# lucastrefezza/quadruplet-sentence-transformer

Measured on AMD Instinct MI355X. Metric: quadruplets/sec (seq_len=128, all-MiniLM-L6-v2) training step, higher is better.
Workload: dtype bf16; 1 GPU; all-MiniLM-L6-v2 dims (random-init), 64 quadruplets/GPU x 1 GPU, seq_len=128, fwd + gamma-quadruplet loss + bwd + clip + AdamW, dropout 0.1 on hidden states and attention probabilities as the reference's train() mode (BASELINE.json configs[1]); global_batch=64, seq_len=128, parallelism=dp1, precision=bf16 MFMA operands, fp32 accumulate/residual/LN/softmax/loss/optimizer, launch=eager

## Files before the change

include/qst_kernels.h:

```cpp
#pragma once
#include <stddef.h>
#include <stdint.h>

#ifdef __cplusplus
extern "C" {
#endif

enum {
    QST_EPI_BF16 = 0,
    QST_EPI_F32_RESID = 1,
    QST_EPI_GELU = 2,
    QST_EPI_GELU_BWD = 3,
    QST_EPI_F32_RESID_BF16 = 4,
    QST_EPI_GELU_MX = 5,
    QST_EPI_GELU_MX_TRAIN = 6
};

typedef struct {
    const uint32_t* state;
    uint32_t site;
    uint32_t thr16;
} QstDrop;
#define QST_DROP_SITE_EMBED 0xE0u
#define QST_DROP_SITE_ATTN_OUT(layer) (4u * (uint32_t)(layer) + 0u)
// ... 73 lines not shown
    int32_t order;
} QstTnGroup;
int qst_gemm_tn_group(const QstTnGroup* grp, void* stream);
int qst_tn_group_ranges(const QstTnGroup* grp, int32_t* row_begin);

int qst_gemm8_stagger(int cycles);
int qst_gemm8_ln_store(int mode);
int qst_gemm_nt8_supported(const QstGemmArgs* a, int epi);
int qst_gemm_nt8(const QstGemmArgs* a, int epi, int tile, void* stream);
int qst_gemm_tn8_group(const QstTnGroup* grp, void* stream);
int qst_gemm_nt8_f8(const QstGemmArgs* a, int epi, int tile, void* stream);
int qst_gemm8_mode(int mode);

int qst_embed_ln_fwd(const int64_t* ids, const int64_t* type_ids, const int32_t* pos_ids,
                     const float* word_emb, const float* pos_emb, const float* type_emb,
                     const float* gamma, const float* beta, float eps, int M, int H,
                     float* y, void* y_bf16, void* xhat_bf16, float* rstd, void* stream);
int qst_embed_ln_fwd_drop(const int64_t* ids, const int64_t* type_ids, const int32_t* pos_ids,
                          const float* word_emb, const float* pos_emb, const float* type_emb,
                          const float* gamma, const float* beta, float eps, int M, int H,
                          float* y, void* y_bf16, void* xhat_bf16, float* rstd, const QstDrop* drop, void* stream);
int qst_ln_fwd(const float* s, const float* gamma, const float* beta, float eps, int M, int H,
               float* y, void* y_bf16, void* xhat_bf16, float* rstd, void* stream);
int qst_ln_fwd_mx(const float* s, const float* gamma, const float* beta, float eps, int M, int H,
                  float* y, void* y_bf16, void* yq, void* ys, void* stream);
int qst_embed_ln_fwd_mx(const int64_t* ids, const int64_t* type_ids, const int32_t* pos_ids,
                        const float* word_emb, const float* pos_emb, const float* type_emb,
                        const float* gamma, const float* beta, float eps, int M, int H,
                        float* y, void* y_bf16, void* yq, void* ys, void* stream);
int qst_ln_fwd_mx_train(const float* s, const float* gamma, const float* beta, float eps, int M, int H, float* y,
                        void* y_bf16, void* xhat_bf16, float* rstd, void* yq, void* ys, void* stream);
int qst_embed_ln_fwd_mx_train(const int64_t* ids, const int64_t* type_ids, const int32_t* pos_ids,
                              const float* word_emb, const float* pos_emb, const float* type_emb,
                              const float* gamma, const float* beta, float eps, int M, int H, float* y,
                              void* y_bf16, void* xhat_bf16, float* rstd, void* yq, void* ys,
                              const QstDrop* drop , void* stream);
size_t qst_ln_bwd_scratch_bytes(int M, int H);
int qst_ln_bwd(const float* dy, const void* xhat_bf16, const float* rstd, const float* gamma, int M, int H,
               float* ds, void* ds_bf16, float* dgamma, float* dbeta, float* scratch, void* stream);
int qst_ln_bwd_drop(const float* dy, const void* xhat_bf16, const float* rstd, const float* gamma, int M, int H,
                    float* ds, void* ds_bf16, float* dgamma, float* dbeta, float* scratch,
                    const QstDrop* drop_in, const QstDrop* drop_out, void* stream);
#define QST_LN_BATCH_MAX 32
typedef struct {
    int32_t count, H, nblocks;
    const float* partials[QST_LN_BATCH_MAX];
    float* dgamma[QST_LN_BATCH_MAX];
    float* dbeta[QST_LN_BATCH_MAX];
    int32_t nblocks_each[QST_LN_BATCH_MAX];
} QstLnReduceBatch;
int qst_ln_bwd_reduce_batch(const QstLnReduceBatch* b, void* stream);
int qst_embed_bwd(const float* ds, const int64_t* ids, const int64_t* type_ids, const int32_t* pos_ids,
                  int nseq, int L, int H, int num_types, float* dword, float* dpos, float* dtype_, void* stream);
int qst_position_ids(const int64_t* ids, int nseq, int L, int arch, int pad_id, int32_t* pos_ids, void* stream);
int qst_forward_prologue(const int64_t* ids, int nseq, int L, int arch, int pad_id, int32_t* pos_ids,
                         uint32_t* drop_state, uint32_t* drop_snapshot, void* stream);

#define QST_POOL_CLS 1
#define QST_POOL_MAX 2
#define QST_POOL_MEAN 4
#define QST_POOL_MEAN_SQRT 8
#define QST_POOL_WMEAN 16
#define QST_POOL_ALL 31
int qst_pool_fwd(const float* tok, const int64_t* mask, int nseq, int L, int H, int mode, int normalize,
                 float* emb, float* pooled, int32_t* argmax, void* stream);
int qst_pool_bwd(const float* demb, const float* pooled, const int32_t* argmax, const int64_t* mask, int nseq, int L, int H,
                 int mode, int normalize, float* dtok, void* stream);

int qst_attention_fwd(const void* qkv, const int64_t* mask, const float* rel_pos, int nseq, int L, int A, int d,
                      void* ctx, float* lse, void* stream);
int qst_attention_bwd(const void* qkv, const void* ctx, const void* dctx, const float* lse, const int64_t* mask,
                      const float* rel_bias, int nseq, int L, int A, int d, void* dqkv, float* drel,
                      float* delta_scratch, void* stream);
typedef struct {
    const void* qkv; const int64_t* mask; const float* rel_pos;
    int32_t nseq, L, A, d;
    void* ctx; float* lse;
    const void* dctx; void* dqkv; float* drel; float* delta_scratch;
    int32_t force_split;
    QstDrop drop;
} QstAttnDesc;
int qst_attention_fwd_ex(const QstAttnDesc* a, void* stream);
int qst_attention_bwd_ex(const QstAttnDesc* a, void* stream);

int qst_rel_bucket_host(int rel, int num_buckets, int max_distance);
int qst_rel_bias_fwd(const float* table, const int32_t* lut, int A, int L, float* rel_bias, void* stream);
int qst_rel_bias_bwd(const float* drel, const int32_t* lut, int buckets, int A, int L, float* dtable, void* stream);
int qst_rel_pos_fwd(const float* table, const int32_t* lut, int A, int L, float* rel_pos, void* stream);
int qst_rel_pos_bwd(const float* drel_pos, const int32_t* lut, int buckets, int A, int L, float* dtable, void* stream);

int qst_gemm_nt_x3(const QstGemmArgs* a, int epi, void* stream);
int qst_gemm_tn_x3(const QstGemmArgs* a, void* stream);
int qst_attention_fwd_x3(const float* qkv, const int64_t* mask, const float* rel_bias, int nseq, int L, int A, int d,
                         float* ctx, void* stream);
int qst_attention_fwd_x3_drop(const float* qkv, const int64_t* mask, const float* rel_bias, int nseq, int L, int A, int d,
                              float* ctx, const QstDrop* drop, void* stream);
int qst_transpose_f32(const float* src, int R, int C, int ld_src, float* dst, int ld_dst, void* stream);
int qst_gelu_f32(const float* u, int64_t n, float* h, void* stream);
int qst_gelu_bwd_f32(const float* dh, const float* u, int64_t n, float* du, void* stream);
int qst_colsum_f32(const float* x, int M, int N, int ld, float* out, void* stream);
int qst_embed_sum_f32(const int64_t* ids, const int64_t* type_ids, const int32_t* pos_ids, const float* word_emb,
                      const float* pos_emb, const float* type_emb, int M, int H, float* s, void* stream);
int qst_ln_bwd_f32(const float* dy, const float* prenorm, const float* gamma, float eps, int M, int H, float* ds,
                   float* dgamma, float* dbeta, void* stream);
int qst_attention_bwd_f32(const float* qkv, const float* ctx, const float* dctx, const int64_t* mask, const float* rel_bias,
                          int nseq, int L, int A, int d, float* dqkv, float* drel_bias, void* stream);
int qst_attention_bwd_f32_drop(const float* qkv, const float* ctx, const float* dctx, const int64_t* mask, const float* rel_bias,
                               int nseq, int L, int A, int d, float* dqkv, float* drel_bias, const QstDrop* drop, void* stream);
size_t qst_attention_bwd_x3_scratch_bytes(int nseq, int L, int A);
int qst_attention_bwd_x3(const float* qkv, const float* ctx, const float* dctx, const int64_t* mask, const float* rel_bias,
                         int nseq, int L, int A, int d, float* dqkv, float* drel_bias, void* scratch, const QstDrop* drop,
                         void* stream);
int qst_dropout_apply_f32(const QstDrop* d, const float* in, const float* resid, int64_t n, float* out, void* stream);

int qst_topk_rows(const float* scores, int64_t ld, const int64_t* index_map, int nrows, int n, int k,
                  float* out_scores, int64_t* out_index, void* stream);

int qst_topk_merge_rows(const float* scores, int64_t ld, int nrows, int n, int64_t col_base, int64_t row_base,
                        int exclude_self, float max_score, int k, float* run_scores, int64_t* run_index, void* stream);

size_t qst_topk_stream_workspace_bytes(int nq, int chunk, int dim);
int qst_topk_stream(const float* queries, const float* corpus, int nq, int nc, int dim, int k, int mode, int chunk,
                    int64_t query_base, int64_t corpus_base, int exclude_self, float max_score,
                    float* run_scores, int64_t* run_index, void* workspace, size_t workspace_bytes, void* stream);

size_t qst_community_workspace_bytes(int n, int chunk, int dim);
int qst_community_count(const float* emb, int n, int dim, float threshold, int chunk, int32_t* counts,
                        uint8_t* self_member, void* workspace, size_t workspace_bytes, void* stream);
int qst_community_members(const float* emb, int n, int dim, float threshold, int chunk, int row0, const int64_t* begin,
                          const int32_t* capacity, int32_t* out_index, float* out_score, int32_t* written,
                          void* workspace, size_t workspace_bytes, void* stream);
int qst_community_claim(const int64_t* begin, const int32_t* len, int ncand, const int32_t* members, int n,
                        uint8_t* taken, uint8_t* accepted, void* stream);
int qst_community_rescore(const float* emb, int n, int dim, const int32_t* rows_a, const int32_t* rows_b, int64_t count,
                          double* out, void* stream);

int qst_shadow_all(const float* params, void* shadow, const int64_t* table_dev, int nseg, int nblocks, void* stream);
int qst_shadow_matrix(const float* src, int rows, int cols, void* dst_bf16, void* dstT_bf16, void* stream);

int qst_gemm_nt_f16(const QstGemmArgs* a, int epi, void* stream);
int qst_gemm_nt_ln_f16(const QstGemmArgs* a, const QstLnEpi* ln, int mode, void* stream);
int qst_gemm_nt8_ln_supported_f16(int N);
int qst_gemm_nt8_ln_block_rows_f16(int M, int N);
int qst_gemm_nt8_ln_f16(const QstGemmArgs* a, const QstLnEpi* ln, int mode, void* stream);
int qst_gemm_nt8_ln_timeouts_f16(void);
int qst_ffn_chain_f16(const QstFfnArgs* a, const QstLnEpi* ln, int mode, void* stream);
int qst_gemm_tn_f16(const QstGemmArgs* a, void* stream);
int qst_gemm_tn_group_f16(const QstTnGroup* grp, void* stream);
int qst_gemm_nt8_supported_f16(const QstGemmArgs* a, int epi);
int qst_gemm_nt8_f16(const QstGemmArgs* a, int epi, int tile, void* stream);
int qst_gemm_tn8_group_f16(const QstTnGroup* grp, void* stream);
int qst_embed_ln_fwd_f16(const int64_t* ids, const int64_t* type_ids, const int32_t* pos_ids,
                         const float* word_emb, const float* pos_emb, const float* type_emb,
                         const float* gamma, const float* beta, float eps, int M, int H,
                         float* y, void* y_f16, void* xhat_f16, float* rstd, void* stream);
int qst_embed_ln_fwd_drop_f16(const int64_t* ids, const int64_t* type_ids, const int32_t* pos_ids,
                              const float* word_emb, const float* pos_emb, const float* type_emb,
                              const float* gamma, const float* beta, float eps, int M, int H,
                              float* y, void* y_f16, void* xhat_f16, float* rstd, const QstDrop* drop, void* stream);
int qst_ln_fwd_f16(const float* s, const float* gamma, const float* beta, float eps, int M, int H,
                   float* y, void* y_f16, void* xhat_f16, float* rstd, void* stream);
int qst_ln_bwd_f16(const float* dy, const void* xhat_f16, const float* rstd, const float* gamma, int M, int H,
                   float* ds, void* ds_f16, float* dgamma, float* dbeta, float* scratch, void* stream);
int qst_ln_bwd_drop_f16(const float* dy, const void* xhat_f16, const float* rstd, const float* gamma, int M, int H,
                        float* ds, void* ds_f16, float* dgamma, float* dbeta, float* scratch,
                        const QstDrop* drop_in, const QstDrop* drop_out, void* stream);
// ... 18 lines not shown
```

quadruplet-sentence-transformer_amd/_lib.py:

```python
from __future__ import annotations

import ctypes as C
import os
from typing import Optional

_HERE = os.path.dirname(os.path.abspath(__file__))
LIB_PATH = os.path.join(_HERE, "libqst.so")

c_i64p = C.POINTER(C.c_int64)
c_i32p = C.POINTER(C.c_int32)
c_f32p = C.POINTER(C.c_float)
vp = C.c_void_p


class QstError(RuntimeError):
    pass


class QstConfig(C.Structure):
    _fields_ = [("arch", C.c_int32), ("vocab_size", C.c_int32), ("hidden_size", C.c_int32),
                ("num_layers", C.c_int32), ("num_heads", C.c_int32), ("intermediate_size", C.c_int32),
                ("max_position", C.c_int32), ("type_vocab_size", C.c_int32), ("layer_norm_eps", C.c_float),
                ("normalize", C.c_int32), ("rel_buckets", C.c_int32), ("rel_max_distance", C.c_int32),
                ("pad_token_id", C.c_int32), ("precision", C.c_int32)]
# ... 69 lines not shown
                                vp]),
    "qst_mnrl_nested_workspace_bytes": (C.c_size_t, [C.c_int, C.c_int, C.c_int, C.c_int]),
    "qst_mnrl_nested_loss": (C.c_int, [vp, vp, C.c_int, C.c_int, C.c_int, c_i32p, c_f32p, C.c_int, C.c_float, C.c_int, vp, vp,
                                       vp, vp, vp, vp, C.c_size_t, vp]),
    "qst_batch_triplet_workspace_bytes": (C.c_size_t, [C.c_int, C.c_int]),
    "qst_batch_triplet_loss": (C.c_int, [vp, vp, C.c_int, C.c_int, C.c_int, C.c_int, C.c_float, vp, vp, vp, vp, vp, C.c_size_t,
                                         vp]),
    "qst_cosent_workspace_bytes": (C.c_size_t, [C.c_int, C.c_int]),
    "qst_cosent_loss": (C.c_int, [vp, vp, vp, C.c_int, C.c_int, C.c_int, C.c_float, vp, vp, vp, vp, vp, vp, C.c_size_t, vp]),
    "qst_embed_mse": (C.c_int, [vp, vp, C.c_int, C.c_int, vp, vp, vp, vp, vp]),
    "qst_margin_mse_loss": (C.c_int, [vp, vp, vp, vp, C.c_int, C.c_int, C.c_int, C.c_int, vp, vp, vp, vp, vp, vp, vp, vp]),
    "qst_clip_adamw_step": (C.c_int, [vp, vp, vp, vp, vp, C.c_float, C.c_float, C.c_float, C.c_float, C.c_float,
                                      C.c_float, C.c_float, C.c_int64, vp, vp, vp]),
    "qst_clip_adamw_step_joint": (C.c_int, [vp, vp, vp, vp, vp, vp, vp, vp, vp, vp, C.c_int64, C.c_float, C.c_float, C.c_float,
                                            C.c_float, C.c_float, C.c_float, C.c_float, C.c_int64, vp, vp, vp]),
    "qst_softmax_head_fwd": (C.c_int, [vp, vp, vp, vp, C.c_int, C.c_int, C.c_int, C.c_int, vp, vp]),
    "qst_softmax_head_bwd_workspace_bytes": (C.c_size_t, [C.c_int, C.c_int, C.c_int, C.c_int]),
    "qst_softmax_head_bwd": (C.c_int, [vp, vp, vp, vp, C.c_int, C.c_int, C.c_int, C.c_int, vp, vp, vp, vp, vp, C.c_size_t, vp]),
    "qst_dense_head_fwd": (C.c_int, [vp, C.c_int, vp, vp, C.c_int, C.c_int, C.c_int, C.c_int, C.c_int, vp, vp, vp]),
    "qst_dense_head_bwd_workspace_bytes": (C.c_size_t, [C.c_int, C.c_int, C.c_int]),
    "qst_dense_head_bwd": (C.c_int, [vp, C.c_int, vp, vp, vp, vp, C.c_int, C.c_int, C.c_int, C.c_int, C.c_int, vp, vp, vp, vp,
                                     C.c_size_t, vp]),
    "qst_softmax_ce": (C.c_int, [vp, vp, C.c_int, C.c_int, C.c_int64, C.c_int, vp, vp, vp, vp, vp, vp]),
    "qst_binary_eval_workspace_bytes": (C.c_size_t, [C.c_int64, C.c_int]),
    "qst_binary_eval": (C.c_int, [vp, vp, C.c_int64, C.c_int, c_i32p, vp, vp, C.c_size_t, vp]),
    "qst_rerank_scores": (C.c_int, [vp, vp, vp, C.c_int64, C.c_int64, C.c_int, C.c_int, vp, vp]),
    "qst_rerank_workspace_bytes": (C.c_size_t, [C.c_int64, C.c_int64]),
    "qst_rerank_metrics": (C.c_int, [vp, vp, vp, C.c_int64, C.c_int64, C.c_int, vp, vp, vp, C.c_size_t, vp]),
    "qst_shadow8_bytes": (C.c_int64, [C.POINTER(QstConfig)]),
    "qst_clip_adamw_step_sched": (C.c_int, [vp, vp, vp, vp, vp, C.c_float, C.c_float, C.c_float, C.c_float, C.c_float,
                                            C.c_float, C.c_float, C.c_int64, C.c_int64, vp, vp, vp, vp]),
    "qst_topk_workspace_bytes": (C.c_size_t, [C.c_int, C.c_int, C.c_int]),
    "qst_topk_scores": (C.c_int, [vp, vp, C.c_int, C.c_int, C.c_int, C.c_int, C.c_int, vp, vp, vp, C.c_size_t, vp]),
    "qst_topk_scores_capped": (C.c_int, [vp, vp, C.c_int, C.c_int, C.c_int, C.c_int, C.c_int, C.c_float, vp, vp, vp,
                                         C.c_size_t, vp]),
    "qst_score_workspace_bytes": (C.c_size_t, [C.c_int, C.c_int, C.c_int]),
    "qst_score_matrix": (C.c_int, [vp, vp, C.c_int, C.c_int, C.c_int, C.c_int, vp, C.c_int64, vp, C.c_size_t, vp]),
    "qst_gemm_nt": (C.c_int, [C.POINTER(QstGemmArgs), C.c_int, vp]),
    "qst_gemm_nt_f8": (C.c_int, [C.POINTER(QstGemmArgs), C.c_int, vp]),
    "qst_quant_mx": (C.c_int, [vp, C.c_int, C.c_int64, C.c_int, vp, vp, vp]),
    "qst_gemm_nt_ln_supported": (C.c_int, [C.c_int]),
    "qst_gemm_nt_ln": (C.c_int, [C.POINTER(QstGemmArgs), C.POINTER(QstLnEpi), C.c_int, vp]),
    "qst_gemm_nt_ln_block_rows": (C.c_int, [C.c_int]),
    "qst_gemm_nt_ln_block_rows_m": (C.c_int, [C.c_int, C.c_int]),
    "qst_gemm_nt8_ln_block_rows": (C.c_int, [C.c_int, C.c_int]),
    "qst_gemm8_stagger": (C.c_int, [C.c_int]),
    "qst_gemm8_ln_store": (C.c_int, [C.c_int]),
    "qst_gemm_nt8_ln_supported": (C.c_int, [C.c_int]),
    "qst_gemm_nt8_ln": (C.c_int, [C.POINTER(QstGemmArgs), C.POINTER(QstLnEpi), C.c_int, vp]),
    "qst_gemm_nt8_ln_timeouts": (C.c_int, []),
    "qst_gemm_nt8_f8_ln": (C.c_int, [C.POINTER(QstGemmArgs), C.POINTER(QstLnEpi), vp]),
    "qst_ffn_chain_supported": (C.c_int, [C.c_int, C.c_int]),
    "qst_ffn_chain": (C.c_int, [C.POINTER(QstFfnArgs), C.POINTER(QstLnEpi), C.c_int, vp]),
    "qst_gemm_tn": (C.c_int, [C.POINTER(QstGemmArgs), vp]),
    "qst_gemm_tn_group": (C.c_int, [C.POINTER(QstTnGroup), vp]),
    "qst_tn_group_ranges": (C.c_int, [C.POINTER(QstTnGroup), c_i32p]),
    "qst_gemm_nt8_supported": (C.c_int, [C.POINTER(QstGemmArgs), C.c_int]),
    "qst_gemm_nt8": (C.c_int, [C.POINTER(QstGemmArgs), C.c_int, C.c_int, vp]),
    "qst_gemm_tn8_group": (C.c_int, [C.POINTER(QstTnGroup), vp]),
    "qst_gemm_nt8_f8": (C.c_int, [C.POINTER(QstGemmArgs), C.c_int, C.c_int, vp]),
    "qst_gemm8_mode": (C.c_int, [C.c_int]),
    "qst_embed_ln_fwd": (C.c_int, [vp, vp, vp, vp, vp, vp, vp, vp, C.c_float, C.c_int, C.c_int, vp, vp, vp, vp, vp]),
    "qst_embed_ln_fwd_drop": (C.c_int, [vp, vp, vp, vp, vp, vp, vp, vp, C.c_float, C.c_int, C.c_int, vp, vp, vp, vp,
                                        C.POINTER(QstDrop), vp]),
    "qst_ln_fwd_mx": (C.c_int, [vp, vp, vp, C.c_float, C.c_int, C.c_int, vp, vp, vp, vp, vp]),
    "qst_embed_ln_fwd_mx": (C.c_int, [vp, vp, vp, vp, vp, vp, vp, vp, C.c_float, C.c_int, C.c_int, vp, vp, vp, vp, vp]),
    "qst_ln_fwd_mx_train": (C.c_int, [vp, vp, vp, C.c_float, C.c_int, C.c_int, vp, vp, vp, vp, vp, vp, vp]),
    "qst_embed_ln_fwd_mx_train": (C.c_int, [vp, vp, vp, vp, vp, vp, vp, vp, C.c_float, C.c_int, C.c_int, vp, vp, vp, vp, vp, vp,
                                            vp, vp]),
    "qst_ln_fwd": (C.c_int, [vp, vp, vp, C.c_float, C.c_int, C.c_int, vp, vp, vp, vp, vp]),
    "qst_ln_bwd_scratch_bytes": (C.c_size_t, [C.c_int, C.c_int]),
    "qst_ln_bwd_reduce_batch": (C.c_int, [vp, vp]),
    "qst_ln_bwd": (C.c_int, [vp, vp, vp, vp, C.c_int, C.c_int, vp, vp, vp, vp, vp, vp]),
    "qst_ln_bwd_drop": (C.c_int, [vp, vp, vp, vp, C.c_int, C.c_int, vp, vp, vp, vp, vp, C.POINTER(QstDrop), C.POINTER(QstDrop), vp]),
    "qst_embed_bwd": (C.c_int, [vp, vp, vp, vp, C.c_int, C.c_int, C.c_int, C.c_int, vp, vp, vp, vp]),
    "qst_position_ids": (C.c_int, [vp, C.c_int, C.c_int, C.c_int, C.c_int, vp, vp]),
    "qst_forward_prologue": (C.c_int, [vp, C.c_int, C.c_int, C.c_int, C.c_int, vp, vp, vp, vp]),
    "qst_pool_fwd": (C.c_int, [vp, vp, C.c_int, C.c_int, C.c_int, C.c_int, C.c_int, vp, vp, vp, vp]),
    "qst_pool_bwd": (C.c_int, [vp, vp, vp, vp, C.c_int, C.c_int, C.c_int, C.c_int, C.c_int, vp, vp]),
    "qst_attention_fwd": (C.c_int, [vp, vp, vp, C.c_int, C.c_int, C.c_int, C.c_int, vp, vp, vp]),
    "qst_attention_bwd": (C.c_int, [vp, vp, vp, vp, vp, vp, C.c_int, C.c_int, C.c_int, C.c_int, vp, vp, vp, vp]),
    "qst_attention_fwd_ex": (C.c_int, [C.POINTER(QstAttnDesc), vp]),
    "qst_attention_bwd_ex": (C.c_int, [C.POINTER(QstAttnDesc), vp]),
    "qst_dropout_multipliers": (C.c_int, [C.POINTER(QstDrop), C.c_int, C.c_int64, vp, vp]),
    "qst_abi_sizeof": (C.c_int64, [C.c_int]),
    "qst_normalize_rows": (C.c_int, [vp, C.c_int, C.c_int, vp, vp]),
    "qst_cls_head_fwd": (C.c_int, [vp, C.c_int64, C.c_int, C.c_int, vp, vp, vp, vp, C.c_int, C.c_int, C.c_int, vp, vp]),
    "qst_dropout_init": (C.c_int, [vp, C.c_uint64, vp]),
    "qst_dropout_advance": (C.c_int, [vp, vp]),
    "qst_encoder_set_dropout": (C.c_int, [vp, C.c_float, C.c_float, vp]),
    "qst_encoder_set_ffn_chain": (C.c_int, [vp, C.c_int]),
    "qst_encoder_set_ln_fusion": (C.c_int, [vp, C.c_int]),
    "qst_encoder_set_wgrad_pairs": (C.c_int, [vp, C.c_int]),
    "qst_wgrad_pairs_rule": (C.c_int, [C.POINTER(QstConfig), C.c_int]),
    "qst_wgrad_tiles": (C.c_int, [C.POINTER(QstConfig), C.c_int, C.c_int]),
    "qst_encoder_set_pooling": (C.c_int, [vp, C.c_int]),
    "qst_encoder_embedding_dim": (C.c_int, [vp]),
    "qst_transpose_f32": (C.c_int, [vp, C.c_int, C.c_int, C.c_int, vp, C.c_int, vp]),
    "qst_gelu_f32": (C.c_int, [vp, C.c_int64, vp, vp]),
    "qst_gelu_bwd_f32": (C.c_int, [vp, vp, C.c_int64, vp, vp]),
    "qst_colsum_f32": (C.c_int, [vp, C.c_int, C.c_int, C.c_int, vp, vp]),
    "qst_embed_sum_f32": (C.c_int, [vp, vp, vp, vp, vp, vp, C.c_int, C.c_int, vp, vp]),
    "qst_ln_bwd_f32": (C.c_int, [vp, vp, vp, C.c_float, C.c_int, C.c_int, vp, vp, vp, vp]),
    "qst_attention_bwd_f32": (C.c_int, [vp, vp, vp, vp, vp, C.c_int, C.c_int, C.c_int, C.c_int, vp, vp, vp]),
    "qst_attention_bwd_f32_drop": (C.c_int, [vp, vp, vp, vp, vp, C.c_int, C.c_int, C.c_int, C.c_int, vp, vp, vp, vp]),
    "qst_attention_bwd_x3_scratch_bytes": (C.c_size_t, [C.c_int, C.c_int, C.c_int]),
    "qst_attention_bwd_x3": (C.c_int, [vp, vp, vp, vp, vp, C.c_int, C.c_int, C.c_int, C.c_int, vp, vp, vp, vp, vp]),
    "qst_dropout_apply_f32": (C.c_int, [vp, vp, vp, C.c_int64, vp, vp]),
    "qst_comm_unique_id": (C.c_int, [vp]),
    "qst_comm_init": (C.c_int, [C.c_int, C.c_int, vp, C.POINTER(vp)]),
    "qst_allreduce_bucket": (C.c_int, [vp, vp, C.c_int64, C.c_int, vp]),
    "qst_comm_rank": (C.c_int, [vp]),
    "qst_comm_world": (C.c_int, [vp]),
    "qst_comm_destroy": (None, [vp]),
    "qst_comm_last_error": (C.c_char_p, []),
    "qst_rel_bucket_host": (C.c_int, [C.c_int, C.c_int, C.c_int]),
    "qst_rel_bias_fwd": (C.c_int, [vp, vp, C.c_int, C.c_int, vp, vp]),
    "qst_rel_bias_bwd": (C.c_int, [vp, vp, C.c_int, C.c_int, C.c_int, vp, vp]),
    "qst_rel_pos_fwd": (C.c_int, [vp, vp, C.c_int, C.c_int, vp, vp]),
    "qst_rel_pos_bwd": (C.c_int, [vp, vp, C.c_int, C.c_int, C.c_int, vp, vp]),
    "qst_topk_rows": (C.c_int, [vp, C.c_int64, vp, C.c_int, C.c_int, C.c_int, vp, vp, vp]),
    "qst_topk_merge_rows": (C.c_int, [vp, C.c_int64, C.c_int, C.c_int, C.c_int64, C.c_int64, C.c_int, C.c_float, C.c_int,
                                      vp, vp, vp]),
    "qst_topk_stream_workspace_bytes": (C.c_size_t, [C.c_int, C.c_int, C.c_int]),
    "qst_topk_stream": (C.c_int, [vp, vp, C.c_int, C.c_int, C.c_int, C.c_int, C.c_int, C.c_int, C.c_int64, C.c_int64,
                                  C.c_int, C.c_float, vp, vp, vp, C.c_size_t, vp]),
    "qst_community_workspace_bytes": (C.c_size_t, [C.c_int, C.c_int, C.c_int]),
    "qst_community_count": (C.c_int, [vp, C.c_int, C.c_int, C.c_float, C.c_int, vp, vp, vp, C.c_size_t, vp]),
    "qst_community_members": (C.c_int, [vp, C.c_int, C.c_int, C.c_float, C.c_int, C.c_int, vp, vp, vp, vp, vp, vp,
                                        C.c_size_t, vp]),
    "qst_community_claim": (C.c_int, [vp, vp, C.c_int, vp, C.c_int, vp, vp, vp]),
    "qst_community_rescore": (C.c_int, [vp, C.c_int, C.c_int, vp, vp, C.c_int64, vp, vp]),
    "qst_shadow_matrix": (C.c_int, [vp, C.c_int, C.c_int, vp, vp, vp]),
    "qst_shadow_all": (C.c_int, [vp, vp, vp, C.c_int, C.c_int, vp]),
    "qst_gemm_nt_x3": (C.c_int, [C.POINTER(QstGemmArgs), C.c_int, vp]),
    "qst_gemm_tn_x3": (C.c_int, [C.POINTER(QstGemmArgs), vp]),
    "qst_attention_fwd_x3": (C.c_int, [vp, vp, vp, C.c_int, C.c_int, C.c_int, C.c_int, vp, vp]),
    "qst_attention_fwd_x3_drop": (C.c_int, [vp, vp, vp, C.c_int, C.c_int, C.c_int, C.c_int, vp, vp, vp]),
}

F16_TWINS = ["qst_gemm_nt", "qst_gemm_nt_ln", "qst_gemm_nt8_ln_supported", "qst_gemm_nt8_ln_block_rows", "qst_gemm_nt8_ln", "qst_gemm_nt8_ln_timeouts", "qst_ffn_chain", "qst_gemm_tn", "qst_gemm_tn_group", "qst_gemm_nt8_supported",
             "qst_gemm_nt8", "qst_gemm_tn8_group", "qst_embed_ln_fwd", "qst_embed_ln_fwd_drop", "qst_ln_fwd", "qst_ln_bwd",
             "qst_ln_bwd_drop", "qst_attention_fwd", "qst_attention_bwd", "qst_attention_fwd_ex", "qst_attention_bwd_ex",
             "qst_shadow_all", "qst_shadow_matrix"]
for _n in F16_TWINS:
    SIGNATURES[_n + "_f16"] = SIGNATURES[_n]
SIGNATURES["qst_shadow_all_split_f16"] = (C.c_int, [vp, vp, vp, vp, C.c_int, C.c_int, vp])
SIGNATURES["qst_amp_scaler_init"] = (C.c_int, [vp, C.c_float, vp])
SIGNATURES["qst_clip_adamw_step_amp"] = (C.c_int, [vp, vp, vp, vp, vp, C.c_float, C.c_float, C.c_float, C.c_float, C.c_float,
                                                  C.c_float, C.c_float, C.c_int64, C.c_int64, vp, vp, C.c_float, C.c_float,
                                                  C.c_int32, vp, vp, vp])

_lib: Optional[C.CDLL] = None


def load() -> C.CDLL:
    global _lib
    if _lib is not None:
        return _lib
    if not os.path.exists(LIB_PATH):
        raise QstError(f"HIP extension not built: {LIB_PATH} is missing (no CPU fallback exists). "
                       f"Run `make -C {os.path.join(_HERE, 'csrc')}` or __graft_entry__.build().")
    import torch
    lib = C.CDLL(LIB_PATH)
    for name, (res, args) in SIGNATURES.items():
        fn = getattr(lib, name)
# ... 32 lines not shown
```

quadruplet-sentence-transformer_amd/csrc/attention.hip:

```cpp
#include <stdlib.h>
#include "qst_common.h"
#include "qst_kernels.h"

namespace {

constexpr float kMaskMin = -3.4028234663852886e38f;
constexpr float kLog2e = 1.4426950408889634f;
constexpr float kMaskLog2 = -3.0e38f;

template <int D> __device__ __forceinline__ uint32_t rr_off(int row, int chunk) {
    if (D == 32) return (uint32_t)(row * 64 + ((chunk ^ ((row >> 2) & 3)) << 4));
    return (uint32_t)(row * 128 + ((chunk ^ ((row >> 1) & 7)) << 4));
}
template <int D> __device__ __forceinline__ uint32_t tr_off(int row, int byte) {
    if (D == 32) return (uint32_t)(row * 64 + byte);
    return (uint32_t)(row * 128 + (byte ^ (((row >> 1) & 1) << 6)));
}
__device__ __forceinline__ op16x4 lds_tr(const char* p) {
    return lds_tr16_op(p);
}
template <int D> __device__ __forceinline__ op16x8 tr_frag(const char* img, int row0, int ddb, int lane) {
    const int li = lane & 15, q = li >> 2, p = li & 3, gsel = (lane >> 4) & 1, h = lane >> 5;
    const int byte = ddb * 64 + gsel * 32 + 8 * p;
    const op16x4 a = lds_tr(img + tr_off<D>(row0 + 4 * h + q, byte));
// ... 914 lines not shown
                        *(u32x2*)(dsimg + ds_off(32 * wave + fr, (it * 32 + 8 * g + 4 * h) * 2)) = pkd;
                    }
                    if (REL && a.drel) {
                        float lo = 0.f, hi = 0.f;
#pragma unroll
                        for (int r = 0; r < 16; ++r) diag_add(s[r], r, lane, lo, hi);
                        diag_store(drel_s + wave * 2 * L, L, j0, i0, lane, lo, hi);
                    }
#pragma unroll
                    for (int ks = 0; ks < 2; ++ks) {
                        const op16x8 pf = acc_frag(dp, ks), sf = acc_frag(s, ks);
#pragma unroll
                        for (int b = 0; b < DB; ++b) {
                            const op16x8 dt = tr_frag_rr64(dimg, it * 32 + 16 * ks, b, lane);
                            const op16x8 qt = tr_frag_rr64(qimg, it * 32 + 16 * ks, b, lane);
                            dv[b] = mfma32_op(dt, pf, dv[b]);
                            dk[b] = mfma32_op(qt, sf, dk[b]);
                        }
                    }
                }
            }
            __syncthreads();
            if (qt_mine * 32 < rows) {
                const int li = lane & 15, q = li >> 2, pp = li & 3, gsel = (lane >> 4) & 1;
                const int byte = qt_mine * 64 + gsel * 32 + 8 * pp;
                auto accumulate = [&](f32x16& acc) {
                    for (int ks = 0; ks < nkeys / 16; ++ks) {
                        const op16x4 lo = lds_tr(dsimg + ds_off(16 * ks + 4 * h + q, byte));
                        const op16x4 hi = lds_tr(dsimg + ds_off(16 * ks + 8 + 4 * h + q, byte));
                        op16x8 df;
#pragma unroll
                        for (int e = 0; e < 4; ++e) { df[e] = lo[e]; df[4 + e] = hi[e]; }
                        const op16x8 kt = tr_frag_rr64(kimg, 16 * ks, b_mine, lane);
                        acc = mfma32_op(kt, df, acc);
                    }
                };
                if (c == 0) accumulate(dq[0]);
                if (NC > 1 && c == 1) accumulate(dq[1]);
                if (NC > 2 && c == 2) accumulate(dq[2]);
                if (NC > 3 && c == 3) accumulate(dq[3]);
            }
        }
        if (active) {
            op16* krow = a.dqkv + qkv_base(a, seq, head, D) + (size_t)kj * ld + a.woff;
            op16* vrow = krow + a.woff;
#pragma unroll
            for (int b = 0; b < DB; ++b)
#pragma unroll
                for (int g = 0; g < 4; ++g) {
                    u32x2 pk;
                    pk[0] = pack_op2(dk[b][4 * g] * a.scale, dk[b][4 * g + 1] * a.scale);
                    pk[1] = pack_op2(dk[b][4 * g + 2] * a.scale, dk[b][4 * g + 3] * a.scale);
                    *(u32x2*)(krow + b * 32 + 8 * g + 4 * h) = pk;
                    pk[0] = pack_op2(dv[b][4 * g], dv[b][4 * g + 1]);
                    pk[1] = pack_op2(dv[b][4 * g + 2], dv[b][4 * g + 3]);
                    *(u32x2*)(vrow + b * 32 + 8 * g + 4 * h) = pk;
                }
        }
    }
#pragma unroll
    for (int c = 0; c < NC; ++c) {
        const int qi = c * 128 + qt_mine * 32 + fr;
        if (c >= nchunk || qi >= L) continue;
        op16* orow = a.dqkv + qkv_base(a, seq, head, D) + (size_t)qi * ld + b_mine * 32;
#pragma unroll
        for (int g = 0; g < 4; ++g) {
            u32x2 pk;
            pk[0] = pack_op2(dq[c][4 * g] * a.scale, dq[c][4 * g + 1] * a.scale);
            pk[1] = pack_op2(dq[c][4 * g + 2] * a.scale, dq[c][4 * g + 3] * a.scale);
            *(u32x2*)(orow + 8 * g + 4 * h) = pk;
        }
    }
    if (REL && a.drel) {
        __syncthreads();
        for (int t = tid; t < 2 * L; t += 512) {
            float v = 0.f;
#pragma unroll
            for (int w = 0; w < 8; ++w) v += drel_s[w * 2 * L + t];
            if (v != 0.f) atomicAdd(a.drel + (size_t)head * 2 * L + t, v);
        }
    }
}

template <typename K>
int set_lds(K kern, size_t bytes) {
    QST_HIP_CHECK(hipFuncSetAttribute((const void*)kern, hipFuncAttributeMaxDynamicSharedMemorySize, (int)bytes));
    return QST_OK;
}

}

static int check_attn(int nseq, int L, int A, int d) {
    if (nseq <= 0 || L <= 0 || A <= 0) return QST_ERR_BAD_ARG;
    if ((d != 32 && d != 64) || (L % 32) != 0 || L > 512) return QST_ERR_UNSUPPORTED;
    return QST_OK;
}

static int fill_args(const QstAttnDesc* q, AttnArgs& a) {
    if (!q || !q->qkv || !q->mask || !q->ctx) return QST_ERR_BAD_ARG;
    if (int rc = check_attn(q->nseq, q->L, q->A, q->d)) return rc;
    a.qkv = (const op16*)q->qkv; a.mask = q->mask; a.rel = q->rel_pos;
    a.nseq = q->nseq; a.L = q->L; a.A = q->A; a.H = q->A * q->d; a.scale = 1.0f / sqrtf((float)q->d);
    a.ld = 3 * a.H; a.woff = a.H;
    a.drop = q->drop;
    if (a.drop.thr16 > 65535u) return QST_ERR_BAD_ARG;
    if (!a.drop.state) a.drop.thr16 = 0u;
    if (a.drop.thr16 && (int64_t)q->nseq * q->A * q->L * q->L >= ((int64_t)1 << 32)) return QST_ERR_UNSUPPORTED;
    return QST_OK;
}

extern "C" int QST_K(qst_attention_fwd_ex)(const QstAttnDesc* q, void* stream) {
    AttnArgs a{};
    if (int rc = fill_args(q, a)) return rc;
    a.out = (op16*)q->ctx; a.lse_out = q->lse;
    const int nseq = a.nseq, L = a.L, A = a.A, d = q->d;
    const bool rel = a.rel != nullptr, drop = a.drop.thr16 != 0u;
    int rc;
    const int grid = nseq * A * ((L + 127) / 128);
    const size_t lds = (size_t)2 * 128 * d * 2 + (((size_t)L * 4 + 15) & ~(size_t)15) + (size_t)4 * 32 * d * 2 +
                       (rel ? (size_t)2 * L * 4 : 0);
    hipStream_t st = (hipStream_t)stream;
#define QST_FWD(D_, DR_) do { if ((rc = set_lds(attn_fwd_kernel<D_, DR_>, lds))) return rc; \
                              attn_fwd_kernel<D_, DR_><<<grid, 256, lds, st>>>(a); } while (0)
    if (d == 32) { if (drop) QST_FWD(32, true); else QST_FWD(32, false); }
    else         { if (drop) QST_FWD(64, true); else QST_FWD(64, false); }
#undef QST_FWD
    QST_LAUNCH_CHECK();
    return QST_OK;
}

extern "C" int QST_K(qst_attention_bwd_ex)(const QstAttnDesc* q, void* stream) {
    AttnArgs a{};
    if (int rc = fill_args(q, a)) return rc;
    if (!q->dctx || !q->lse || !q->dqkv || !q->delta_scratch) return QST_ERR_BAD_ARG;
    if (q->drel && !q->rel_pos) return QST_ERR_BAD_ARG;
    a.ctx = (const op16*)q->ctx; a.dctx = (const op16*)q->dctx; a.lse_in = q->lse;
    a.dqkv = (op16*)q->dqkv; a.drel = q->drel; a.delta = q->delta_scratch;
    const int nseq = a.nseq, L = a.L, A = a.A, d = q->d;
    const bool rel = a.rel != nullptr, drop = a.drop.thr16 != 0u;
    int rc;
    const int grid = nseq * A * ((L + 127) / 128);
    const size_t lds_q = (size_t)3 * 128 * d * 2 + (((size_t)L + 3) & ~(size_t)3) * 4 + (rel ? (size_t)2 * L * 4 : 0);
    const size_t lds_kv = (size_t)4 * 128 * d * 2 + 256 * 4 + (rel ? (size_t)10 * L * 4 : 0);
    hipStream_t st = (hipStream_t)stream;
#define QST_RUN(K_, G_, LDS_) do { if ((rc = set_lds(K_, LDS_))) return rc; K_<<<G_, 256, LDS_, st>>>(a); QST_LAUNCH_CHECK(); } while (0)
    const bool fits32 = (int64_t)nseq * L * 3 * A * d * 2 < 0x7FFFFF00LL;
    if (L <= 128 && d == 32 && !q->force_split && fits32) {
        const size_t lds_f = (size_t)5 * 128 * d * 2 + DS_IMG + 256 * 4 + (rel ? (size_t)10 * L * 4 : 0);
        const int gf = min(nseq * A, 512);
        if (rel) { if (drop) QST_RUN((attn_bwd_fused_kernel<32, true, true>), gf, lds_f); else QST_RUN((attn_bwd_fused_kernel<32, true, false>), gf, lds_f); }
        else     { if (drop) QST_RUN((attn_bwd_fused_kernel<32, false, true>), gf, lds_f); else QST_RUN((attn_bwd_fused_kernel<32, false, false>), gf, lds_f); }
        return QST_OK;
    }
    static const bool env_pair = [] { const char* e = getenv("QST_ATTN_BWD_PAIR"); return e && e[0] == '1'; }();
    const bool one64_auto = !q->force_split && !env_pair;
    if (d == 64 && (q->force_split == 2 || one64_auto)) {
        const size_t lds_o = (size_t)131072 + (size_t)2 * L * 4 + (rel ? (size_t)18 * L * 4 : 0);
        if (lds_o <= 163840) {
            const int go = nseq * A;
#define QST_ONE(NC_) do { \
            if (rel) { if (drop) QST_RUN512((attn_bwd_one64_kernel<NC_, true, true>), go, lds_o); else QST_RUN512((attn_bwd_one64_kernel<NC_, true, false>), go, lds_o); } \
            else     { if (drop) QST_RUN512((attn_bwd_one64_kernel<NC_, false, true>), go, lds_o); else QST_RUN512((attn_bwd_one64_kernel<NC_, false, false>), go, lds_o); } } while (0)
#define QST_RUN512(K_, G_, LDS_) do { if ((rc = set_lds(K_, LDS_))) return rc; K_<<<G_, 512, LDS_, st>>>(a); QST_LAUNCH_CHECK(); } while (0)
            if (L <= 256) QST_ONE(2); else if (L <= 384) QST_ONE(3); else QST_ONE(4);
#undef QST_RUN512
#undef QST_ONE
            return QST_OK;
        }
    }
    if (d == 32) {
        if (drop) QST_RUN((attn_bwd_dq_kernel<32, true>), grid, lds_q); else QST_RUN((attn_bwd_dq_kernel<32, false>), grid, lds_q);
        if (rel) { if (drop) QST_RUN((attn_bwd_dkv_kernel<32, true, true>), grid, lds_kv); else QST_RUN((attn_bwd_dkv_kernel<32, true, false>), grid, lds_kv); }
        else     { if (drop) QST_RUN((attn_bwd_dkv_kernel<32, false, true>), grid, lds_kv); else QST_RUN((attn_bwd_dkv_kernel<32, false, false>), grid, lds_kv); }
    } else {
        if (drop) QST_RUN((attn_bwd_dq_kernel<64, true>), grid, lds_q); else QST_RUN((attn_bwd_dq_kernel<64, false>), grid, lds_q);
        if (rel) { if (drop) QST_RUN((attn_bwd_dkv_kernel<64, true, true>), grid, lds_kv); else QST_RUN((attn_bwd_dkv_kernel<64, true, false>), grid, lds_kv); }
        else     { if (drop) QST_RUN((attn_bwd_dkv_kernel<64, false, true>), grid, lds_kv); else QST_RUN((attn_bwd_dkv_kernel<64, false, false>), grid, lds_kv); }
    }
#undef QST_RUN
    return QST_OK;
}

extern "C" int QST_K(qst_attention_fwd)(const void* qkv, const int64_t* mask, const float* rel_bias, int nseq, int L, int A,
                                 int d, void* ctx, float* lse, void* stream) {
    QstAttnDesc q{};
    q.qkv = qkv; q.mask = mask; q.rel_pos = rel_bias; q.nseq = nseq; q.L = L; q.A = A; q.d = d; q.ctx = ctx; q.lse = lse;
    return QST_K(qst_attention_fwd_ex)(&q, stream);
}
extern "C" int QST_K(qst_attention_bwd)(const void* qkv, const void* ctx, const void* dctx, const float* lse,
                                 const int64_t* mask, const float* rel_bias, int nseq, int L, int A, int d,
                                 void* dqkv, float* drel, float* delta_scratch, void* stream) {
    QstAttnDesc q{};
    q.qkv = qkv; q.mask = mask; q.rel_pos = rel_bias; q.nseq = nseq; q.L = L; q.A = A; q.d = d; q.ctx = (void*)ctx;
    q.lse = (float*)lse; q.dctx = dctx; q.dqkv = dqkv; q.drel = drel; q.delta_scratch = delta_scratch;
    return QST_K(qst_attention_bwd_ex)(&q, stream);
}

#if !QST_OP_F16
extern "C" int qst_debug_attn_occupancy(int which, int lds_bytes) {
    int n = -1;
    if (which == 0) (void)hipOccupancyMaxActiveBlocksPerMultiprocessor(&n, attn_fwd_kernel<32>, 256, lds_bytes);
    if (which == 1) (void)hipOccupancyMaxActiveBlocksPerMultiprocessor(&n, attn_bwd_dq_kernel<32>, 256, lds_bytes);
    if (which == 2) (void)hipOccupancyMaxActiveBlocksPerMultiprocessor(&n, attn_bwd_dkv_kernel<32, false>, 256, lds_bytes);
    return n;
// ... 3 lines not shown
```

Baseline: 14360 quadruplets/s.

## Add persistent single-pass attention forward kernel for d=32 with cross-item prefetch

Adds a persistent attention forward kernel specialised for head dim 32 and L<=128. Its grid is capped at three workgroups per CU, and each workgroup loops over (sequence, head) items, prefetching the next item's Q/K/V and mask into registers while it computes the current one. Fully unmasked 32-key tiles skip the mask add. The goal is to cut launch and tail overhead and hide global load latency. The trade-off is extra register pressure and a new code path, used only when there is no relative position bias and split is not forced.

```diff
diff --git a/include/qst_kernels.h b/include/qst_kernels.h
--- a/include/qst_kernels.h
+++ b/include/qst_kernels.h
@@ -179,6 +179,7 @@
 } QstAttnDesc;
 int qst_attention_fwd_ex(const QstAttnDesc* a, void* stream);
 int qst_attention_bwd_ex(const QstAttnDesc* a, void* stream);
+int qst_attention_fwd_grid(int nseq, int A, int L);
 
 int qst_rel_bucket_host(int rel, int num_buckets, int max_distance);
 int qst_rel_bias_fwd(const float* table, const int32_t* lut, int A, int L, float* rel_bias, void* stream);
diff --git a/quadruplet-sentence-transformer_amd/_lib.py b/quadruplet-sentence-transformer_amd/_lib.py
--- a/quadruplet-sentence-transformer_amd/_lib.py
+++ b/quadruplet-sentence-transformer_amd/_lib.py
@@ -175,6 +175,7 @@
     "qst_attention_bwd": (C.c_int, [vp, vp, vp, vp, vp, vp, C.c_int, C.c_int, C.c_int, C.c_int, vp, vp, vp, vp]),
     "qst_attention_fwd_ex": (C.c_int, [C.POINTER(QstAttnDesc), vp]),
     "qst_attention_bwd_ex": (C.c_int, [C.POINTER(QstAttnDesc), vp]),
+    "qst_attention_fwd_grid": (C.c_int, [C.c_int, C.c_int, C.c_int]),
     "qst_dropout_multipliers": (C.c_int, [C.POINTER(QstDrop), C.c_int, C.c_int64, vp, vp]),
     "qst_abi_sizeof": (C.c_int64, [C.c_int]),
     "qst_normalize_rows": (C.c_int, [vp, C.c_int, C.c_int, vp, vp]),
diff --git a/quadruplet-sentence-transformer_amd/csrc/attention.hip b/quadruplet-sentence-transformer_amd/csrc/attention.hip
--- a/quadruplet-sentence-transformer_amd/csrc/attention.hip
+++ b/quadruplet-sentence-transformer_amd/csrc/attention.hip
@@ -1020,6 +1020,273 @@
     }
 }
 
+#ifndef QST_ATTN_ONE_PASS
+#define QST_ATTN_ONE_PASS 0
+#endif
+constexpr int kFwdOneWgsPerCu = 3;
+constexpr int kFwdOneLds = 2 * 128 * 32 * 2 + 128 * 4 + 4 * 32 * 32 * 2;
+
+template <bool DROP, bool MASKED>
+__device__ __forceinline__ void fwd_one_tile_online(const char* kimg, const char* vimg, const float* madd, const op16x8 (&qf)[2],
+                                                    int jt, int lane, float sc2, const DropCtx& dc, uint32_t dword0,
+                                                    f32x16& o, float& m, float& l) {
+    const int h = lane >> 5, fr = lane & 31;
+    f32x16 s;
+#pragma unroll
+    for (int r = 0; r < 16; ++r) s[r] = 0.f;
+#pragma unroll
+    for (int ks = 0; ks < 2; ++ks) {
+        const op16x8 kf = *(const op16x8*)(kimg + rr_off<32>(jt * 32 + fr, 2 * ks + h));
+        s = mfma32_op(kf, qf[ks], s);
+    }
+    const int j0 = jt * 32;
+    float mx = -INFINITY;
+#pragma unroll
+    for (int r = 0; r < 16; ++r) {
+        float v = __builtin_fmaf(s[r], sc2, MASKED ? madd[j0 + acc_row(r, h)] : 0.f);
+        s[r] = v;
+        mx = fmaxf(mx, v);
+    }
+    mx = fmaxf(mx, swap32(mx));
+    const float mn = fmaxf(m, mx);
+    const float alpha = __builtin_amdgcn_exp2f(m - mn);
+    float ps = 0.f;
+#pragma unroll
+    for (int r = 0; r < 16; ++r) { s[r] = __builtin_amdgcn_exp2f(s[r] - mn); ps += s[r]; }
+    ps += swap32(ps);
+    l = l * alpha + ps;
+    m = mn;
+    if (DROP && dc.thr) {
+#pragma unroll
+        for (int r = 0; r < 16; r += 4) {
+            const uint32_t w = drop_word4(dc, dword0 + (uint32_t)(j0 + 8 * (r >> 2)));
+            if (!drop_keep_byte<0>(dc, w)) s[r] = 0.f;
+            if (!drop_keep_byte<1>(dc, w)) s[r + 1] = 0.f;
+            if (!drop_keep_byte<2>(dc, w)) s[r + 2] = 0.f;
+            if (!drop_keep_byte<3>(dc, w)) s[r + 3] = 0.f;
+        }
+    }
+#pragma unroll
+    for (int r = 0; r < 16; ++r) o[r] *= alpha;
+#pragma unroll
+    for (int ks = 0; ks < 2; ++ks) {
+        const op16x8 pf = acc_frag(s, ks);
+        const op16x8 vf = tr_frag<32>(vimg, jt * 32 + 16 * ks, 0, lane);
+        o = mfma32_op(vf, pf, o);
+    }
+}
+
+__device__ __forceinline__ void fwd_one_scale_masked(f32x16& s, const float* madd, int jt, int h, float sc2, float& mx) {
+#pragma unroll
+    for (int g = 0; g < 4; ++g) {
+        const f32x4 ma = *(const f32x4*)(madd + jt * 32 + 8 * g + 4 * h);
+#pragma unroll
+        for (int e = 0; e < 4; e += 2) {
+            f32x2 v, mv;
+            v[0] = s[4 * g + e]; v[1] = s[4 * g + e + 1];
+            mv[0] = ma[e]; mv[1] = ma[e + 1];
+            v = v * sc2 + mv;
+            s[4 * g + e] = v[0]; s[4 * g + e + 1] = v[1];
+            mx = fmaxf(fmaxf(mx, v[0]), v[1]);
+        }
+    }
+}
+typedef __attribute__((ext_vector_type(2))) short s16x2;
+template <bool DROP>
+__device__ __forceinline__ void fwd_one_tile_pv(const char* vimg, const f32x16& s, int jt, int lane, float tsc, float negm,
+                                                const DropCtx& dc, uint32_t dword0, f32x16& o, f32x2& ps) {
+    uint32_t pw[8];
+#pragma unroll
+    for (int r = 0; r < 16; r += 2) {
+        f32x2 v;
+        v[0] = s[r]; v[1] = s[r + 1];
+        v = v * tsc + negm;
+        v[0] = __builtin_amdgcn_exp2f(v[0]);
+        v[1] = __builtin_amdgcn_exp2f(v[1]);
+        ps += v;
+        pw[r >> 1] = pack_op2(v[0], v[1]);
+    }
+    if (DROP) {
+        const short kk = (short)(0x8000u - dc.thr);
+        const s16x2 kk2 = {kk, kk};
+#pragma unroll
+        for (int g = 0; g < 4; ++g) {
+            const uint32_t w = qst_hash32(((dword0 >> 2) + (uint32_t)(jt * 8 + 2 * g)) ^ dc.key);
+            const s16x2 k01 = (__builtin_bit_cast(s16x2, __builtin_amdgcn_perm(0u, w, 0x0c010c00u)) + kk2) >> 15;
+            const s16x2 k23 = (__builtin_bit_cast(s16x2, __builtin_amdgcn_perm(0u, w, 0x0c030c02u)) + kk2) >> 15;
+            pw[2 * g] &= __builtin_bit_cast(uint32_t, k01);
+            pw[2 * g + 1] &= __builtin_bit_cast(uint32_t, k23);
+        }
+    }
+#pragma unroll
+    for (int ks = 0; ks < 2; ++ks) {
+        u32x4 pu = {pw[4 * ks], pw[4 * ks + 1], pw[4 * ks + 2], pw[4 * ks + 3]};
+        const op16x8 pf = __builtin_bit_cast(op16x8, pu);
+        const op16x8 vf = tr_frag<32>(vimg, jt * 32 + 16 * ks, 0, lane);
+        o = mfma32_op(vf, pf, o);
+    }
+}
+
+template <bool DROP, int NT>
+__global__ __launch_bounds__(256, kFwdOneWgsPerCu) void attn_fwd_one_kernel(AttnArgs a) {
+    op_saturate(true);
+    extern __shared__ __attribute__((aligned(16))) char smem[];
+    constexpr int D = 32, KS = 2, IMG = 128 * D * 2, CPR = D / 8, PER = 128 * CPR / 256;
+    char* kimg = smem;
+    char* vimg = smem + IMG;
+    float* madd = (float*)(smem + 2 * IMG);
+    char* ostg = smem + 2 * IMG + 128 * 4;
+    const int tid = threadIdx.x, lane = tid & 63, h = lane >> 5, fr = lane & 31;
+    const int wave = __builtin_amdgcn_readfirstlane(tid >> 6);
+    const int ld = a.ld, rows = NT * 32;
+    const int i0 = wave * 32, qi = i0 + fr;
+    const bool active = i0 < rows;
+    const int nitems = a.nseq * a.A;
+    const float sc2 = a.scale * kLog2e;
+    constexpr uint32_t kOob = 0x7FFFFFF0u;
+    const __amdgpu_buffer_rsrc_t rq = make_rsrc(a.qkv, (uint32_t)((size_t)a.nseq * a.L * ld * 2));
+    const __amdgpu_buffer_rsrc_t ro = make_rsrc(a.out, (uint32_t)((size_t)a.nseq * a.L * a.H * 2));
+    uint32_t vkv[PER], vq[KS];
+#pragma unroll
+    for (int k = 0; k < PER; ++k) {
+        const int idx = tid + 256 * k, row = idx / CPR, c = idx % CPR;
+        vkv[k] = row < rows ? (uint32_t)(row * ld + c * 8) * 2u : kOob;
+    }
+#pragma unroll
+    for (int s = 0; s < KS; ++s) vq[s] = active ? (uint32_t)(qi * ld + 16 * s + 8 * h) * 2u : kOob;
+    const __amdgpu_buffer_rsrc_t rm = make_rsrc(a.mask, (uint32_t)((size_t)a.nseq * a.L * 8));
+    const __amdgpu_buffer_rsrc_t rl = make_rsrc(a.lse_out, (uint32_t)((size_t)nitems * a.L * 4));
+    const uint32_t vm0 = lane < rows ? (uint32_t)lane * 8u : kOob, vm1 = lane + 64 < rows ? (uint32_t)(lane + 64) * 8u : kOob;
+
+    u32x4 pq[KS], pk[PER], pv[PER];
+    u32x2 nm0 = {1u, 0u}, nm1 = {1u, 0u};
+    auto prefetch = [&](int item, int part) {
+        const int head = item % a.A, seq = item / a.A;
+        const uint32_t sq = (uint32_t)(qkv_base(a, seq, head, D) * 2);
+        const uint32_t wb = (uint32_t)(a.woff * 2);
+        if (part < 0 || part == 0) {
+#pragma unroll
+            for (int k = 0; k < PER; ++k) pk[k] = __builtin_amdgcn_raw_buffer_load_b128(rq, (int)vkv[k], (int)(sq + wb), 0);
+        }
+        if (part < 0 || part == 1) {
+#pragma unroll
+            for (int k = 0; k < PER; ++k) pv[k] = __builtin_amdgcn_raw_buffer_load_b128(rq, (int)vkv[k], (int)(sq + 2 * wb), 0);
+        }
+        if (part < 0 || part == 2) {
+#pragma unroll
+            for (int s = 0; s < KS; ++s) pq[s] = __builtin_amdgcn_raw_buffer_load_b128(rq, (int)vq[s], (int)sq, 0);
+            nm0 = __builtin_amdgcn_raw_buffer_load_b64(rm, (int)vm0, (int)((uint32_t)seq * a.L * 8u), 0);
+            nm1 = __builtin_amdgcn_raw_buffer_load_b64(rm, (int)vm1, (int)((uint32_t)seq * a.L * 8u), 0);
+        }
+    };
+
+    const int half = gridDim.x >> 1;
+    const bool paired = (a.A % 2 == 0) && (gridDim.x % 16 == 0);
+    const int bsub = paired ? ((int)blockIdx.x >= half) : 0;
+    const int bp = paired ? (int)blockIdx.x - bsub * half : (int)blockIdx.x;
+    const int stride = paired ? half : (int)gridDim.x;
+    const int nunits = paired ? nitems / 2 : nitems;
+    auto item_of = [&](int unit) { return paired ? 2 * unit + bsub : unit; };
+    const DropCtx dc = DROP ? drop_ctx8(a.drop) : DropCtx{0u, 0u, 1.f};
+    const uint32_t dlane = (uint32_t)qi * a.L + 4u * h;
+
+    int unit = bp;
+    if (unit < nunits) prefetch(item_of(unit), -1);
+    for (; unit < nunits; unit += stride) {
+        const int item = item_of(unit);
+        const int head = item % a.A, seq = item / a.A;
+        const uint32_t dword0 = (uint32_t)item * a.L * a.L + dlane;
+        __syncthreads();
+#pragma unroll
+        for (int k = 0; k < PER; ++k) {
+            const int idx = tid + 256 * k, row = idx / CPR, c = idx % CPR;
+            *(u32x4*)(kimg + rr_off<D>(row, c)) = pk[k];
+            *(u32x4*)(vimg + tr_off<D>(row, c * 16)) = pv[k];
+        }
+        const bool keep0 = lane >= rows || (nm0[0] | nm0[1]) != 0u, keep1 = lane + 64 >= rows || (nm1[0] | nm1[1]) != 0u;
+        if (wave == 0) {
+            madd[lane] = keep0 ? 0.f : kMaskLog2;
+            madd[lane + 64] = keep1 ? 0.f : kMaskLog2;
+        }
+        const uint64_t b0 = __ballot(keep0), b1 = __ballot(keep1);
+        const bool full[4] = {(uint32_t)b0 == 0xFFFFFFFFu, (uint32_t)(b0 >> 32) == 0xFFFFFFFFu,
+                              (uint32_t)b1 == 0xFFFFFFFFu, (uint32_t)(b1 >> 32) == 0xFFFFFFFFu};
+        op16x8 qf[KS];
+#pragma unroll
+        for (int s = 0; s < KS; ++s) qf[s] = __builtin_bit_cast(op16x8, pq[s]);
+        const bool more = unit + stride < nunits;
+        const int next_item = more ? item_of(unit + stride) : 0;
+        __syncthreads();
+
+        f32x16 o;
+#pragma unroll
+        for (int r = 0; r < 16; ++r) o[r] = 0.f;
+        float m = -INFINITY, l = 0.f;
+#if QST_ATTN_ONE_PASS
+        f32x16 s[NT];
+#pragma unroll
+        for (int jt = 0; jt < NT; ++jt) {
+#pragma unroll
+            for (int r = 0; r < 16; ++r) s[jt][r] = 0.f;
+#pragma unroll
+            for (int ks = 0; ks < KS; ++ks) {
+                const op16x8 kf = *(const op16x8*)(kimg + rr_off<D>(jt * 32 + fr, 2 * ks + h));
+                s[jt] = mfma32_op(kf, qf[ks], s[jt]);
+            }
+        }
+#pragma unroll
+        for (int jt = 0; jt < NT; ++jt) {
+            if (full[jt]) {
+                float t = fmaxf(s[jt][0], s[jt][1]);
+#pragma unroll
+                for (int r = 2; r < 16; r += 2) t = fmaxf(fmaxf(t, s[jt][r]), s[jt][r + 1]);
+                m = fmaxf(m, t * sc2);
+            } else {
+                fwd_one_scale_masked(s[jt], madd, jt, h, sc2, m);
+            }
+        }
+        m = fmaxf(m, swap32(m));
+        f32x2 ps = {0.f, 0.f};
+#pragma unroll
+        for (int jt = 0; jt < 3 || jt < NT; ++jt) {
+            if (more && jt < 3) prefetch(next_item, jt);
+            if (jt < NT) fwd_one_tile_pv<DROP>(vimg, s[jt < NT ? jt : 0], jt, lane, full[jt] ? sc2 : 1.0f, -m, dc, dword0, o, ps);
+        }
+        l = ps[0] + ps[1];
+        l += swap32(l);
+#else
+#pragma unroll
+        for (int jt = 0; jt < 3 || jt < NT; ++jt) {
+            if (more && jt < 3) prefetch(next_item, jt);
+            if (jt >= NT) continue;
+            if (full[jt]) fwd_one_tile_online<DROP, false>(kimg, vimg, madd, qf, jt, lane, sc2, dc, dword0, o, m, l);
+            else          fwd_one_tile_online<DROP, true>(kimg, vimg, madd, qf, jt, lane, sc2, dc, dword0, o, m, l);
+        }
+#endif
+        if (!active) continue;
+        const float inv = dc.scale / l;
+        char* stg = ostg + wave * (32 * D * 2);
+#pragma unroll
+        for (int g = 0; g < 4; ++g) {
+            u32x2 pk2;
+            pk2[0] = pack_op2(o[4 * g] * inv, o[4 * g + 1] * inv);
+            pk2[1] = pack_op2(o[4 * g + 2] * inv, o[4 * g + 3] * inv);
+            *(u32x2*)(stg + rr_off<D>(fr, g) + 8 * h) = pk2;
+        }
+        const uint32_t so = (uint32_t)((((size_t)seq * a.L + i0) * a.H + head * D) * 2);
+#pragma unroll
+        for (int kk = 0; kk < 32 * CPR / 64; ++kk) {
+            const int idx = lane + 64 * kk, row = idx / CPR, c = idx % CPR;
+            const u32x4 v = *(const u32x4*)(stg + rr_off<D>(row, c));
+            __builtin_amdgcn_raw_buffer_store_b128(v, ro, (int)((uint32_t)(row * a.H + c * 8) * 2u), (int)so,
+                                                   QST_STREAM_STORES ? 2 : 0);
+        }
+        if (h == 0 && a.lse_out)
+            __builtin_amdgcn_raw_buffer_store_b32(__builtin_bit_cast(uint32_t, (m + __log2f(l)) * 0.6931471805599453f), rl,
+                                                  qi * 4, (int)((uint32_t)item * a.L * 4u), 0);
+    }
+}
+
 template <typename K>
 int set_lds(K kern, size_t bytes) {
     QST_HIP_CHECK(hipFuncSetAttribute((const void*)kern, hipFuncAttributeMaxDynamicSharedMemorySize, (int)bytes));
@@ -1047,6 +1314,25 @@
     return QST_OK;
 }
 
+static int fwd_one_grid(int64_t nseq, int64_t A, int64_t L) {
+    if (nseq <= 0 || A <= 0 || L <= 0) return QST_ERR_BAD_ARG;
+    if (L > 128 || (L % 32) != 0 || nseq * L * 3 * A * 32 * 2 >= 0x7FFFFF00LL) return 0;
+    static int cus[64];
+    int dev = 0;
+    QST_HIP_CHECK(hipGetDevice(&dev));
+    int n = (dev >= 0 && dev < 64) ? cus[dev] : 0;
+    if (n <= 0) {
+        QST_HIP_CHECK(hipDeviceGetAttribute(&n, hipDeviceAttributeMultiprocessorCount, dev));
+        if (n <= 0) return QST_ERR_HIP;
+        if (dev >= 0 && dev < 64) cus[dev] = n;
+    }
+    const int64_t items = nseq * A, resident = (int64_t)kFwdOneWgsPerCu * n;
+    return (int)(items < resident ? items : resident);
+}
+#if !QST_OP_F16
+extern "C" int qst_attention_fwd_grid(int nseq, int A, int L) { return fwd_one_grid(nseq, A, L); }
+#endif
+
 extern "C" int QST_K(qst_attention_fwd_ex)(const QstAttnDesc* q, void* stream) {
     AttnArgs a{};
     if (int rc = fill_args(q, a)) return rc;
@@ -1054,10 +1340,22 @@
     const int nseq = a.nseq, L = a.L, A = a.A, d = q->d;
     const bool rel = a.rel != nullptr, drop = a.drop.thr16 != 0u;
     int rc;
+    hipStream_t st = (hipStream_t)stream;
+    if (d == 32 && !rel && !q->force_split) {
+        const int g1 = fwd_one_grid(nseq, A, L);
+        if (g1 < 0) return g1;
+        if (g1 > 0) {
+#define QST_FWD1(NT_) do { if (drop) attn_fwd_one_kernel<true, NT_><<<g1, 256, kFwdOneLds, st>>>(a); \
+                           else      attn_fwd_one_kernel<false, NT_><<<g1, 256, kFwdOneLds, st>>>(a); } while (0)
+            if (L == 128) QST_FWD1(4); else if (L == 96) QST_FWD1(3); else if (L == 64) QST_FWD1(2); else QST_FWD1(1);
+#undef QST_FWD1
+            QST_LAUNCH_CHECK();
+            return QST_OK;
+        }
+    }
     const int grid = nseq * A * ((L + 127) / 128);
     const size_t lds = (size_t)2 * 128 * d * 2 + (((size_t)L * 4 + 15) & ~(size_t)15) + (size_t)4 * 32 * d * 2 +
                        (rel ? (size_t)2 * L * 4 : 0);
-    hipStream_t st = (hipStream_t)stream;
 #define QST_FWD(D_, DR_) do { if ((rc = set_lds(attn_fwd_kernel<D_, DR_>, lds))) return rc; \
                               attn_fwd_kernel<D_, DR_><<<grid, 256, lds, st>>>(a); } while (0)
     if (d == 32) { if (drop) QST_FWD(32, true); else QST_FWD(32, false); }
```

Measured after the change: 14390 quadruplets/s, median of 4. About the same (+0.2%).
